# suvajit-patra/sl-hwgat

Measured on AMD Instinct MI355X. Metric: clips/sec fwd+bwd at B=64 T=128 J=67; %HBM roofline; 1->8 GPU scaling, higher is better.
Workload: dtype f32

## Files before the change

### sl-hwgat_amd/csrc/gemm_f32_tn256.hip

```cpp
#include <stdlib.h>
#include <type_traits>
#include "common.h"
#include "fused_ops.h"
#include "gemm_f32.h"
#include "gemm_dispatch.h"

namespace {

constexpr int BT = 256, TM = 16, NST = 3;
constexpr int STG = 2 * TM * BT;

constexpr int SG_MFMA = 0x008, SG_VALU = 0x002, SG_VMEM_RD = 0x020, SG_DS_RD = 0x100, SG_DS_WR = 0x200;

template <int NVM = 0>
__device__ __forceinline__ void pin8() {
#pragma unroll
    for (int q = 0; q < 8; ++q) {
        if (q < 4) __builtin_amdgcn_sched_group_barrier(SG_DS_RD, 1, 0);
        if constexpr (NVM > 0) __builtin_amdgcn_sched_group_barrier(SG_VMEM_RD, NVM, 0);
        __builtin_amdgcn_sched_group_barrier(SG_MFMA, 4, 0);
    }
}
template <int NA, int NB>
__device__ __forceinline__ void pin_commit() {
#pragma unroll
    for (int i = 0; i < 4; ++i) {
        if constexpr (NA > 0) __builtin_amdgcn_sched_group_barrier(SG_VALU, NA, 0);
        __builtin_amdgcn_sched_group_barrier(SG_DS_WR, 1, 0);
        __builtin_amdgcn_sched_group_barrier(SG_DS_RD, 1, 0);
        __builtin_amdgcn_sched_group_barrier(SG_MFMA, 4, 0);
        if constexpr (NB > 0) __builtin_amdgcn_sched_group_barrier(SG_VALU, NB, 0);
        __builtin_amdgcn_sched_group_barrier(SG_DS_WR, 1, 0);
        __builtin_amdgcn_sched_group_barrier(SG_MFMA, 4, 0);
    }
}

#ifdef HWGAT_LAB
__device__ unsigned long long* g_tn256_stamps = nullptr;
#define TN256_STAMP(i) do { if (g_tn256_stamps && threadIdx.x == 0) g_tn256_stamps[blockIdx.x * 2 + (i)] = __builtin_amdgcn_s_memtime(); } while (0)
#else
#define TN256_STAMP(i) do {} while (0)
#endif

template <int PRO, bool BLN, bool SLAB = false>
__global__ __launch_bounds__(256, 1) void gemm_tn256_k(TnArgs p, float* __restrict__ ws = nullptr) {
    HWGAT_RESOLVE_SEED1(p);
    __shared__ __attribute__((aligned(16))) float sm[NST * STG];
    const int tid = threadIdx.x, lane = tid & 63, wave = tid >> 6;
    const int lq = lane & 31, hh = lane >> 5;
    const int wn = wave >> 1, wk = wave & 1;
    const int tiles_k = p.K / BT, n_tiles = (p.N / BT) * tiles_k;
    const int xcd = blockIdx.x & 7, j = blockIdx.x >> 3;
    const int tile = j % n_tiles;
    const int split = (j / n_tiles) * 8 + xcd;
    if (split >= p.n_split) return;
    const int n0 = (tile / tiles_k) * BT, k0 = (tile % tiles_k) * BT;
    const int64_t r_begin = (int64_t)split * p.rows_per_split;
    const int64_t r_end = r_begin + p.rows_per_split < p.M ? r_begin + p.rows_per_split : p.M;
    if (r_begin >= r_end) return;
    const int n_it = (int)((r_end - r_begin) / TM);
    TN256_STAMP(0);

    const int lrow = tid >> 6, lc4 = (tid & 63) * 4;
    const uint32_t pro_th = drop_thresh(p.pro_p);
    const float pro_sc = 1.0f / (1.0f - p.pro_p);
    f32x4 ra[2][4], rb[2][4];
    f32x2 bms[2][4];
    f32x4 colsum = {0.f, 0.f, 0.f, 0.f};
    f32x4 lg = {1.f, 1.f, 1.f, 1.f}, lb = {0.f, 0.f, 0.f, 0.f};
    if constexpr (BLN) {
        lg = *reinterpret_cast<const f32x4*>(p.gamma + k0 + lc4);
        lb = *reinterpret_cast<const f32x4*>(p.beta + k0 + lc4);
    }
    int oa[4], ob[4];
#pragma unroll
    for (int i = 0; i < 4; ++i) { oa[i] = ((lrow + 4 * i) * p.N + lc4) * 4; ob[i] = ((lrow + 4 * i) * p.K + lc4) * 4; }
    auto issue = [&](auto QC, int it) {
        constexpr int Q = decltype(QC)::value;
        const int64_t r0 = r_begin + (int64_t)it * TM;
        const auto da = __builtin_amdgcn_make_buffer_rsrc((void*)(p.A + r0 * p.N + n0), 0, 0x7fffffff, 0x00020000);
        const auto db = __builtin_amdgcn_make_buffer_rsrc((void*)(p.B + r0 * p.K + k0), 0, 0x7fffffff, 0x00020000);
#pragma unroll
        for (int i = 0; i < 4; ++i) {
            ra[Q][i] = __builtin_bit_cast(f32x4, __builtin_amdgcn_raw_buffer_load_b128(da, oa[i], 0, 0));
            rb[Q][i] = __builtin_bit_cast(f32x4, __builtin_amdgcn_raw_buffer_load_b128(db, ob[i], 0, 0));
            if constexpr (BLN) {
                const auto dm = __builtin_amdgcn_make_buffer_rsrc((void*)(p.mean + r0), 0, 0x7fffffff, 0x00020000);
                const auto ds = __builtin_amdgcn_make_buffer_rsrc((void*)(p.rstd + r0), 0, 0x7fffffff, 0x00020000);
                bms[Q][i].x = __builtin_bit_cast(float, __builtin_amdgcn_raw_buffer_load_b32(dm, (lrow + 4 * i) * 4, 0, 0));
                bms[Q][i].y = __builtin_bit_cast(float, __builtin_amdgcn_raw_buffer_load_b32(ds, (lrow + 4 * i) * 4, 0, 0));
            }
        }
    };
    auto commit_a = [&](auto QC, int so, int it, float live, int i) {
        constexpr int Q = decltype(QC)::value;
        f32x4 a = ra[Q][i];
        if constexpr (PRO == PRO_DROP) {
            const int64_t r0 = r_begin + (int64_t)it * TM + lrow;
            a *= drop_keep4(p.pro_seed, (uint64_t)(r0 + 4 * i) * p.N + n0 + lc4, pro_th, pro_sc);
        }
        colsum += a * live;
        *reinterpret_cast<f32x4*>(sm + so * STG + (lrow + 4 * i) * BT + lc4) = a;
    };
    auto commit_b = [&](auto QC, int so, int i) {
        constexpr int Q = decltype(QC)::value;
        f32x4 b = rb[Q][i];
        if constexpr (BLN) {
            f32x2 ms = bms[Q][i];
            asm("" : "+v"(ms));
            b = (b - ms.x) * ms.y * lg + lb;
        }
        *reinterpret_cast<f32x4*>(sm + so * STG + TM * BT + (lrow + 4 * i) * BT + lc4) = b;
    };
    auto commit = [&](auto QC, int so, int it, float live) {
#pragma unroll
        for (int i = 0; i < 4; ++i) { commit_a(QC, so, it, live, i); commit_b(QC, so, i); }
    };

    f32x16 acc[4][4];
#pragma unroll
    for (int i = 0; i < 4; ++i)
#pragma unroll
        for (int jj = 0; jj < 4; ++jj)
#pragma unroll
            for (int e = 0; e < 16; ++e) acc[i][jj][e] = 0.f;

    struct Chunk { f32x4 a[2], b[2]; };
    auto fetch1 = [&](Chunk& c, int so, int ch, int j) {
        const int e = j >> 1;
        const int ro = (2 * (2 * ch + e) + hh) * BT + 4 * lq;
        const float* src = sm + so * STG + ((j & 1) ? TM * BT + wk * 128 : wn * 128) + ro;
        const f32x4 v = *reinterpret_cast<const f32x4*>(__builtin_assume_aligned(src, 16));
        if (j & 1) c.b[e] = v; else c.a[e] = v;
    };
    auto fetch = [&](Chunk& c, int so, int ch) {
#pragma unroll
        for (int j = 0; j < 4; ++j) fetch1(c, so, ch, j);
    };
    auto mfma_chunk = [&](const Chunk& c) {
#pragma unroll
        for (int e = 0; e < 2; ++e)
#pragma unroll
            for (int i = 0; i < 4; ++i)
#pragma unroll
                for (int jj = 0; jj < 4; ++jj)
                    acc[i][jj] = __builtin_amdgcn_mfma_f32_32x32x2f32(c.a[e][i], c.b[e][jj], acc[i][jj], 0, 0, 0);
    };
    Chunk c0, c1;
    constexpr int NV_A = PRO == PRO_DROP ? 52 : 5, NV_B = BLN ? 9 : 1;
    auto stage_body = [&](auto PARC, int it, int st, int st1, int st2) {
        constexpr int PAR = decltype(PARC)::value;
        using Q = std::integral_constant<int, PAR>;
        const int it2 = it + 2 < n_it ? it + 2 : n_it - 1;
        const float live = it + 2 < n_it ? 1.0f : 0.0f;
        issue(std::integral_constant<int, PAR ^ 1>{}, it + 3 < n_it ? it + 3 : n_it - 1);
        fetch(c1, st, 1);
        mfma_chunk(c0);
        pin8<BLN ? 2 : 1>();
        __builtin_amdgcn_sched_barrier(0);
        fetch(c0, st, 2);
        mfma_chunk(c1);
        pin8<>();
        __builtin_amdgcn_sched_barrier(0);
#pragma unroll
        for (int i = 0; i < 4; ++i) {
            commit_a(Q{}, st2, it2, live, i);
            fetch1(c1, st, 3, i);
            commit_b(Q{}, st2, i);
        }
        mfma_chunk(c0);
        pin_commit<NV_A, NV_B>();
        __builtin_amdgcn_sched_barrier(0);
        fetch(c0, st1, 0);
        mfma_chunk(c1);
        pin8<>();
        __builtin_amdgcn_sched_barrier(0);
        __syncthreads();
    };
    using P0 = std::integral_constant<int, 0>;
    using P1 = std::integral_constant<int, 1>;

    issue(P0{}, 0);
    commit(P0{}, 0, 0, 1.0f);
    issue(P1{}, 1);
    commit(P1{}, 1, 1, 1.0f);
    issue(P0{}, 2 < n_it ? 2 : n_it - 1);
    __syncthreads();
    fetch(c0, 0, 0);
#pragma nounroll
    for (int it = 0, s0 = 0, s1 = 1, s2 = 2; it < n_it; it += 2) {
        stage_body(P0{}, it, s0, s1, s2);
        stage_body(P1{}, it + 1, s1, s2, s0);
        const int t = s0; s0 = s2; s2 = s1; s1 = t;
    }

    const bool det = p.det_dw != nullptr;
    float* dwo = det ? p.det_dw + (int64_t)split * p.N * p.K : p.dW;
    if constexpr (SLAB) {
        float* slab = ws + ((int64_t)split * n_tiles + tile) * 65536 + wave * 16384 + lane * 4;
#pragma unroll
        for (int i = 0; i < 4; ++i)
#pragma unroll
            for (int jj = 0; jj < 4; ++jj)
#pragma unroll
                for (int q = 0; q < 4; ++q) {
                    const f32x4 v = {acc[i][jj][4 * q], acc[i][jj][4 * q + 1], acc[i][jj][4 * q + 2], acc[i][jj][4 * q + 3]};
                    *reinterpret_cast<f32x4*>(slab + ((i * 4 + jj) * 4 + q) * 256) = v;
                }
    } else {
#pragma unroll
        for (int i = 0; i < 4; ++i)
#pragma unroll
            for (int jj = 0; jj < 4; ++jj)
#pragma unroll
                for (int r = 0; r < 16; ++r) {
                    const int n = n0 + wn * 128 + 4 * crow(r, hh) + i;
                    const int k = k0 + wk * 128 + 4 * lq + jj;
                    HWGAT_TN_ACC(det, dwo, (int64_t)n * p.K + k, acc[i][jj][r]);
                }
    }
    if (p.db != nullptr && k0 == 0) {
        float* red = sm;
        __syncthreads();
        *reinterpret_cast<f32x4*>(red + lrow * BT + lc4) = colsum;
        __syncthreads();
        if (tid < BT) HWGAT_TN_ACC(det, det ? p.det_db + (int64_t)split * p.N : p.db, n0 + tid, red[tid] + red[BT + tid] + red[2 * BT + tid] + red[3 * BT + tid]);
    }
    TN256_STAMP(1);
}

__global__ __launch_bounds__(256) void tn256_reduce_k(const float* __restrict__ ws, float* __restrict__ dW, int n_split,
                                                      int n_tiles, int tiles_k, int K) {
    const int tile = blockIdx.x >> 8;
    const int idx = (blockIdx.x & 255) * 256 + threadIdx.x;
    const float* src = ws + (int64_t)tile * 65536 + idx;
    const int64_t step = (int64_t)n_tiles * 65536;
    float s = 0.f;
    int sp = 0;
    for (; sp + 8 <= n_split; sp += 8) {
        float v[8];
#pragma unroll
        for (int j = 0; j < 8; ++j) v[j] = src[(sp + j) * step];
#pragma unroll
        for (int j = 0; j < 8; ++j) s += v[j];
    }
    for (; sp < n_split; ++sp) s += src[sp * step];
    const int e = idx & 3, lane = (idx >> 2) & 63, q = (idx >> 8) & 3, t = (idx >> 10) & 15, wave = idx >> 14;
    const int i = t >> 2, jj = t & 3, lq = lane & 31, hh = lane >> 5, wn = wave >> 1, wk = wave & 1;
    const int n0 = (tile / tiles_k) * BT, k0 = (tile % tiles_k) * BT;
    dW[(int64_t)(n0 + wn * 128 + 4 * crow(4 * q + e, hh) + i) * K + k0 + wk * 128 + 4 * lq + jj] += s;
}

}

static void tn256_split(int64_t M, int n_tiles, int& n_split, int64_t& rows_per_split) {
    static const int min_rounds = [] { const char* e = lab_env("HWGAT_TN_ROUNDS"); return e ? atoi(e) : 1; }();
    const TnSplit sp = tn_m_split(M, n_tiles, 256, TM, 2 * TM, min_rounds);
    n_split = sp.n_split;
    rows_per_split = sp.rows_per_split;
}

int64_t hwgat_tn256_ws_floats(int64_t M, int N, int K) {
    if (N % BT || K % BT || M % (2 * TM)) return 0;
    const int n_tiles = (N / BT) * (K / BT);
    int n_split;
    int64_t rows;
    tn256_split(M, n_tiles, n_split, rows);
    return (int64_t)n_split * n_tiles * 65536;
}

int hwgat_launch_tn256(TnArgs a, hipStream_t st, float* ws, int64_t ws_floats) {
    if (a.N % BT || a.K % BT || a.M % (2 * TM)) return HWGAT_ESHAPE;
    const int n_tiles = (a.N / BT) * (a.K / BT);
    tn256_split(a.M, n_tiles, a.n_split, a.rows_per_split);
    if (a.det_dw) {
        if (a.n_split > a.det_cap) return HWGAT_ESHAPE;
        ws = nullptr;
    }
    const int grid = ((a.n_split + 7) / 8) * 8 * n_tiles;
    const bool drop = a.pro_p > 0.f, ln = a.mean != nullptr;
    if (drop && ln) return HWGAT_ESHAPE;
    if (ws && ws_floats >= (int64_t)a.n_split * n_tiles * 65536) {
        if (drop) gemm_tn256_k<PRO_DROP, false, true><<<grid, 256, 0, st>>>(a, ws);
        else if (ln) gemm_tn256_k<PRO_NONE, true, true><<<grid, 256, 0, st>>>(a, ws);
        else gemm_tn256_k<PRO_NONE, false, true><<<grid, 256, 0, st>>>(a, ws);
        tn256_reduce_k<<<n_tiles * 256, 256, 0, st>>>(ws, a.dW, a.n_split, n_tiles, a.K / BT, a.K);
        HWGAT_LAUNCH_CHECK();
    }
    if (drop) gemm_tn256_k<PRO_DROP, false><<<grid, 256, 0, st>>>(a);
    else if (ln) gemm_tn256_k<PRO_NONE, true><<<grid, 256, 0, st>>>(a);
    else gemm_tn256_k<PRO_NONE, false><<<grid, 256, 0, st>>>(a);
    HWGAT_LAUNCH_CHECK();
}

#ifdef HWGAT_LAB
extern "C" int hwgat_lab_tn256_stamps(void* buf) {
    return hipMemcpyToSymbol(HIP_SYMBOL(g_tn256_stamps), &buf, sizeof(buf)) == hipSuccess ? 0 : HWGAT_EINVAL;
}
#endif
```

### sl-hwgat_amd/csrc/gemm_f32_tnw.hip

```cpp
#include <type_traits>
#include "common.h"
#include "fused_ops.h"
#include "gemm_f32.h"

namespace {

constexpr int TM = 16, NST = 3;

constexpr int SG_MFMA = 0x008, SG_VMEM_RD = 0x020, SG_DS_RD = 0x100, SG_DS_WR = 0x200;

template <int MPG, int M1, int N1, int M2, int N2>
__device__ __forceinline__ void il8() {
#pragma unroll
    for (int q = 0; q < 8; ++q) {
        __builtin_amdgcn_sched_group_barrier(SG_MFMA, MPG, 0);
        if constexpr (N1 > 0) __builtin_amdgcn_sched_group_barrier(M1, N1, 0);
        if constexpr (N2 > 0) __builtin_amdgcn_sched_group_barrier(M2, N2, 0);
    }
}

template <int TN, int TK, int WN, int PRO, bool BLN>
__global__ __launch_bounds__(256, 1) void gemm_tnw_k(TnArgs p, float* __restrict__ ws) {
    HWGAT_RESOLVE_SEED1(p);
    constexpr int WK = 4 / WN, IN = TN / WN / 32, JK = TK / WK / 32;
    constexpr int NA = TN / 64, NB = TK / 64;
    constexpr int STG = TM * (TN + TK);
    constexpr int CP = (256 % (TN / 4)) == 0 ? 1 : 3;
    static_assert(TN % 64 == 0 && TK % 64 == 0 && (256 * CP) % (TN / 4) == 0, "tile");
    static_assert(!BLN || 256 % (TK / 4) == 0, "LayerNorm on B: one column group per thread");
    static_assert(IN * JK * 16 <= 192 && IN * WN * 32 == TN && JK * WK * 32 == TK, "sub-tile");
    __shared__ __attribute__((aligned(16))) float sm[NST * STG];
    const int tid = threadIdx.x, lane = tid & 63, wave = tid >> 6;
    const int lq = lane & 31, hh = lane >> 5;
    const int wn = wave / WK, wk = wave % WK;
    const int split = blockIdx.x;
    if (split >= p.n_split) return;
    const int64_t r_begin = (int64_t)split * p.rows_per_split;
    const int64_t r_end = r_begin + p.rows_per_split < p.M ? r_begin + p.rows_per_split : p.M;
    if (r_begin >= r_end) return;
    const int n_it = (int)((r_end - r_begin) / TM);

    const uint32_t pro_th = drop_thresh(p.pro_p);
    const float pro_sc = 1.0f / (1.0f - p.pro_p);
    f32x4 ra[2][NA], rb[2][NB];
    float bm[2][NB], bs[2][NB];
    f32x4 colsum[CP];
#pragma unroll
    for (int j = 0; j < CP; ++j) colsum[j] = f32x4{0.f, 0.f, 0.f, 0.f};
    f32x4 lg = {1.f, 1.f, 1.f, 1.f}, lb = {0.f, 0.f, 0.f, 0.f};
    constexpr int BPR = TK / 4;
    if constexpr (BLN) {
        lg = *reinterpret_cast<const f32x4*>(p.gamma + (tid % BPR) * 4);
        lb = *reinterpret_cast<const f32x4*>(p.beta + (tid % BPR) * 4);
    }
    auto issue = [&](auto QC, int it) {
        constexpr int Q = decltype(QC)::value;
        const int64_t r0 = r_begin + (int64_t)it * TM;
        const float* a = p.A + r0 * TN + tid * 4;
        const float* b = p.B + r0 * TK + tid * 4;
#pragma unroll
        for (int i = 0; i < NA; ++i) ra[Q][i] = *reinterpret_cast<const f32x4*>(a + i * 1024);
#pragma unroll
        for (int i = 0; i < NB; ++i) {
            rb[Q][i] = *reinterpret_cast<const f32x4*>(b + i * 1024);
            if constexpr (BLN) {
                const int64_t row = r0 + (tid + 256 * i) / BPR;
                bm[Q][i] = p.mean[row];
                bs[Q][i] = p.rstd[row];
            }
        }
    };
    auto commit = [&](auto QC, int stage, int it, float live) {
        constexpr int Q = decltype(QC)::value;
        float* As = sm + stage * STG + tid * 4;
        float* Bs = As + TM * TN;
        const uint64_t e0 = (uint64_t)(r_begin + (int64_t)it * TM) * TN + tid * 4;
#pragma unroll
        for (int i = 0; i < NA; ++i) {
            f32x4 a = ra[Q][i];
            if constexpr (PRO == PRO_DROP) a *= drop_keep4(p.pro_seed, e0 + i * 1024, pro_th, pro_sc);
            colsum[i % CP] += a * live;
            *reinterpret_cast<f32x4*>(As + i * 1024) = a;
        }
#pragma unroll
        for (int i = 0; i < NB; ++i) {
            f32x4 b = rb[Q][i];
            if constexpr (BLN) b = (b - bm[Q][i]) * bs[Q][i] * lg + lb;
            *reinterpret_cast<f32x4*>(Bs + i * 1024) = b;
        }
    };

    f32x16 acc[IN][JK];
#pragma unroll
    for (int i = 0; i < IN; ++i)
#pragma unroll
        for (int jj = 0; jj < JK; ++jj)
#pragma unroll
            for (int e = 0; e < 16; ++e) acc[i][jj][e] = 0.f;

    struct Chunk { float a[2][IN], b[2][JK]; };
    auto fetch = [&](Chunk& c, int stage, int ch) {
        const float* As = sm + stage * STG + wn * (IN * 32) + lq;
        const float* Bs = sm + stage * STG + TM * TN + wk * (JK * 32) + lq;
#pragma unroll
        for (int e = 0; e < 2; ++e) {
            const int row = 2 * (2 * ch + e) + hh;
#pragma unroll
            for (int i = 0; i < IN; ++i) c.a[e][i] = As[row * TN + 32 * i];
#pragma unroll
            for (int jj = 0; jj < JK; ++jj) c.b[e][jj] = Bs[row * TK + 32 * jj];
        }
    };
    auto mfma_chunk = [&](const Chunk& c) {
#pragma unroll
        for (int e = 0; e < 2; ++e)
#pragma unroll
            for (int i = 0; i < IN; ++i)
#pragma unroll
                for (int jj = 0; jj < JK; ++jj)
                    acc[i][jj] = __builtin_amdgcn_mfma_f32_32x32x2f32(c.a[e][i], c.b[e][jj], acc[i][jj], 0, 0, 0);
    };
    constexpr int MPG = 2 * IN * JK / 8, RPG = (2 * (IN + JK) + 7) / 8;
    constexpr int LPG = (NA + NB + (BLN ? 2 * NB : 0) + 7) / 8, WPG = (NA + NB + 7) / 8;
    static_assert(MPG * 8 == 2 * IN * JK, "MFMAs per chunk");
    Chunk c0, c1;
    auto stage_body = [&](auto PARC, int it) {
        constexpr int PAR = decltype(PARC)::value;
        const int st = it % NST;
        issue(std::integral_constant<int, PAR ^ 1>{}, it + 3 < n_it ? it + 3 : n_it - 1);
        fetch(c1, st, 1);
        mfma_chunk(c0);
        il8<MPG, SG_DS_RD, RPG, SG_VMEM_RD, LPG>();
        __builtin_amdgcn_sched_barrier(0);
        fetch(c0, st, 2);
        mfma_chunk(c1);
        il8<MPG, SG_DS_RD, RPG, 0, 0>();
        __builtin_amdgcn_sched_barrier(0);
        fetch(c1, st, 3);
        mfma_chunk(c0);
        commit(std::integral_constant<int, PAR>{}, (it + 2) % NST, it + 2 < n_it ? it + 2 : n_it - 1, it + 2 < n_it ? 1.0f : 0.0f);
        il8<MPG, SG_DS_RD, RPG, SG_DS_WR, WPG>();
        __builtin_amdgcn_sched_barrier(0);
        fetch(c0, (it + 1) % NST, 0);
        mfma_chunk(c1);
        il8<MPG, SG_DS_RD, RPG, 0, 0>();
        __builtin_amdgcn_sched_barrier(0);
        __syncthreads();
    };
    using P0 = std::integral_constant<int, 0>;
    using P1 = std::integral_constant<int, 1>;

    issue(P0{}, 0);
    commit(P0{}, 0, 0, 1.0f);
    issue(P1{}, 1);
    commit(P1{}, 1, 1, 1.0f);
    issue(P0{}, 2 < n_it ? 2 : n_it - 1);
    __syncthreads();
    fetch(c0, 0, 0);
    for (int it = 0; it < n_it; it += 2) {
        stage_body(P0{}, it);
        stage_body(P1{}, it + 1);
    }

    const bool det = p.det_dw != nullptr;
    if (ws != nullptr) {
        float* slab = ws + (int64_t)split * (TN * TK) + wave * (IN * JK * 1024) + lane * 4;
#pragma unroll
        for (int i = 0; i < IN; ++i)
#pragma unroll
            for (int jj = 0; jj < JK; ++jj)
#pragma unroll
                for (int q = 0; q < 4; ++q) {
                    const f32x4 v = {acc[i][jj][4 * q], acc[i][jj][4 * q + 1], acc[i][jj][4 * q + 2], acc[i][jj][4 * q + 3]};
                    *reinterpret_cast<f32x4*>(slab + ((i * JK + jj) * 4 + q) * 256) = v;
                }
    } else {
        float* dwo = det ? p.det_dw + (int64_t)split * (TN * TK) : p.dW;
#pragma unroll
        for (int i = 0; i < IN; ++i)
#pragma unroll
            for (int jj = 0; jj < JK; ++jj)
#pragma unroll
                for (int r = 0; r < 16; ++r) {
                    const int n = wn * (IN * 32) + i * 32 + crow(r, hh);
                    const int k = wk * (JK * 32) + jj * 32 + lq;
                    HWGAT_TN_ACC(det, dwo, n * TK + k, acc[i][jj][r]);
                }
    }
    if (p.db != nullptr) {
        constexpr int SL = 1024 * CP / TN;
        float* red = sm;
#pragma unroll
        for (int j = 0; j < CP; ++j) *reinterpret_cast<f32x4*>(red + (tid + 256 * j) * 4) = colsum[j];
        __syncthreads();
        for (int c = tid; c < TN; c += 256) {
            float s = 0.f;
#pragma unroll
            for (int q = 0; q < SL; ++q) s += red[q * TN + c];
            HWGAT_TN_ACC(det, det ? p.det_db + (int64_t)split * TN : p.db, c, s);
        }
    }
}

template <int TN, int TK, int WN>
__global__ __launch_bounds__(256) void tnw_reduce_k(const float* __restrict__ ws, float* __restrict__ dW, int n_split) {
    constexpr int WK = 4 / WN, IN = TN / WN / 32, JK = TK / WK / 32;
    const int idx = blockIdx.x * 256 + threadIdx.x;
    const float* src = ws + idx;
    float s = 0.f;
    int sp = 0;
    for (; sp + 8 <= n_split; sp += 8) {
        float v[8];
#pragma unroll
        for (int j = 0; j < 8; ++j) v[j] = src[(int64_t)(sp + j) * (TN * TK)];
#pragma unroll
        for (int j = 0; j < 8; ++j) s += v[j];
    }
    for (; sp < n_split; ++sp) s += src[(int64_t)sp * (TN * TK)];
    const int e = idx & 3, lane = (idx >> 2) & 63, q = (idx >> 8) & 3, t = (idx >> 10) % (IN * JK), wave = idx / (IN * JK * 1024);
    const int i = t / JK, jj = t % JK, lq = lane & 31, hh = lane >> 5, wn = wave / WK, wk = wave % WK;
    dW[(wn * (IN * 32) + i * 32 + crow(4 * q + e, hh)) * TK + wk * (JK * 32) + jj * 32 + lq] += s;
}

void tnw_split(int64_t M, int& n_split, int64_t& rows_per_split) {
    int64_t want = 256;
    const int64_t max_split = M / (TM * 16) > 0 ? M / (TM * 16) : 1;
    if (want > max_split) want = max_split;
    int64_t rows = (M + want - 1) / want;
    rows = (rows + 2 * TM - 1) / (2 * TM) * (2 * TM);
    n_split = (int)((M + rows - 1) / rows);
    rows_per_split = rows;
}

template <int TN, int TK, int WN>
int launch_shape(const TnArgs& a, hipStream_t st, float* ws) {
    const bool drop = a.pro_p > 0.f, ln = a.mean != nullptr;
    if (drop) gemm_tnw_k<TN, TK, WN, PRO_DROP, false><<<a.n_split, 256, 0, st>>>(a, ws);
    else if (ln) gemm_tnw_k<TN, TK, WN, PRO_NONE, true><<<a.n_split, 256, 0, st>>>(a, ws);
    else gemm_tnw_k<TN, TK, WN, PRO_NONE, false><<<a.n_split, 256, 0, st>>>(a, ws);
    if (ws) tnw_reduce_k<TN, TK, WN><<<TN * TK / 256, 256, 0, st>>>(ws, a.dW, a.n_split);
    HWGAT_LAUNCH_CHECK();
}

}

bool hwgat_tnw_takes(int64_t M, int N, int K, float pro_p, const float* mean) {
    if (M <= 0 || M % (2 * TM) || (pro_p > 0.f && mean)) return false;
    if (N == 128 && K == 128) return pro_p == 0.f;
    return (N == 256 && K == 128) || (N == 128 && K == 256) || (N == 384 && K == 128);
}

int64_t hwgat_tnw_ws_floats(int64_t M, int N, int K) {
    if (!hwgat_tnw_takes(M, N, K, 0.f, nullptr)) return 0;
    int n_split;
    int64_t rows;
    tnw_split(M, n_split, rows);
    return (int64_t)n_split * N * K;
}

int hwgat_launch_tnw(TnArgs a, hipStream_t st, float* ws, int64_t ws_floats) {
    if (!hwgat_tnw_takes(a.M, a.N, a.K, a.pro_p, a.mean)) return HWGAT_ESHAPE;
    tnw_split(a.M, a.n_split, a.rows_per_split);
    if (a.det_dw) {
        if (a.n_split > a.det_cap) return HWGAT_ESHAPE;
        ws = nullptr;
    }
    if (ws && ws_floats < (int64_t)a.n_split * a.N * a.K) ws = nullptr;
    if (a.N == 128 && a.K == 128) return launch_shape<128, 128, 2>(a, st, ws);
    if (a.N == 256 && a.K == 128) return launch_shape<256, 128, 2>(a, st, ws);
    if (a.N == 128 && a.K == 256) return launch_shape<128, 256, 2>(a, st, ws);
    return launch_shape<384, 128, 2>(a, st, ws);
}
```

Measured before the change: 662.1.

## Load LN stats once per quad with DPP broadcast; vectorize tnw LDS fragment reads

In the 256-tile TN kernel, the per-row mean/rstd loads are cut from eight scalar loads per stage to two. Each lane loads one value and the values are shared across the quad with DPP broadcasts, and the schedule pins are adjusted to match. In the tnw kernel, global loads move to buffer loads with immediate offsets. The MFMA operand index mapping is permuted so each lane reads contiguous LDS fragments with vector loads, and the dW writeback and reduce indices are remapped to match. This reduces VMEM and LDS instruction counts but adds DPP ops, and the permuted layout could change LDS bank conflicts.

```diff
diff --git a/sl-hwgat_amd/csrc/gemm_f32_tn256.hip b/sl-hwgat_amd/csrc/gemm_f32_tn256.hip
--- a/sl-hwgat_amd/csrc/gemm_f32_tn256.hip
+++ b/sl-hwgat_amd/csrc/gemm_f32_tn256.hip
@@ -12,12 +12,15 @@
 
 constexpr int SG_MFMA = 0x008, SG_VALU = 0x002, SG_VMEM_RD = 0x020, SG_DS_RD = 0x100, SG_DS_WR = 0x200;
 
-template <int NVM = 0>
+template <int NVM = 0, int NX = 0>
 __device__ __forceinline__ void pin8() {
 #pragma unroll
     for (int q = 0; q < 8; ++q) {
         if (q < 4) __builtin_amdgcn_sched_group_barrier(SG_DS_RD, 1, 0);
-        if constexpr (NVM > 0) __builtin_amdgcn_sched_group_barrier(SG_VMEM_RD, NVM, 0);
+        if constexpr (NVM > 0) {
+            if (q < NX) __builtin_amdgcn_sched_group_barrier(SG_VMEM_RD, NVM + 1, 0);
+            else __builtin_amdgcn_sched_group_barrier(SG_VMEM_RD, NVM, 0);
+        }
         __builtin_amdgcn_sched_group_barrier(SG_MFMA, 4, 0);
     }
 }
@@ -32,6 +35,16 @@
         if constexpr (NB > 0) __builtin_amdgcn_sched_group_barrier(SG_VALU, NB, 0);
         __builtin_amdgcn_sched_group_barrier(SG_DS_WR, 1, 0);
         __builtin_amdgcn_sched_group_barrier(SG_MFMA, 4, 0);
+    }
+}
+
+__device__ __forceinline__ float quad_bcast(float v, int i) {
+    const int x = __builtin_bit_cast(int, v);
+    switch (i) {
+        case 0: return __builtin_bit_cast(float, __builtin_amdgcn_update_dpp(0, x, 0x00, 0xf, 0xf, true));
+        case 1: return __builtin_bit_cast(float, __builtin_amdgcn_update_dpp(0, x, 0x55, 0xf, 0xf, true));
+        case 2: return __builtin_bit_cast(float, __builtin_amdgcn_update_dpp(0, x, 0xaa, 0xf, 0xf, true));
+        default: return __builtin_bit_cast(float, __builtin_amdgcn_update_dpp(0, x, 0xff, 0xf, 0xf, true));
     }
 }
 
@@ -65,7 +78,8 @@
     const uint32_t pro_th = drop_thresh(p.pro_p);
     const float pro_sc = 1.0f / (1.0f - p.pro_p);
     f32x4 ra[2][4], rb[2][4];
-    f32x2 bms[2][4];
+    float bmv[2], bsv[2];
+    const int os = (lrow + 4 * (lane & 3)) * 4;
     f32x4 colsum = {0.f, 0.f, 0.f, 0.f};
     f32x4 lg = {1.f, 1.f, 1.f, 1.f}, lb = {0.f, 0.f, 0.f, 0.f};
     if constexpr (BLN) {
@@ -80,16 +94,16 @@
         const int64_t r0 = r_begin + (int64_t)it * TM;
         const auto da = __builtin_amdgcn_make_buffer_rsrc((void*)(p.A + r0 * p.N + n0), 0, 0x7fffffff, 0x00020000);
         const auto db = __builtin_amdgcn_make_buffer_rsrc((void*)(p.B + r0 * p.K + k0), 0, 0x7fffffff, 0x00020000);
+        if constexpr (BLN) {
+            const auto dm = __builtin_amdgcn_make_buffer_rsrc((void*)(p.mean + r0), 0, 0x7fffffff, 0x00020000);
+            const auto ds = __builtin_amdgcn_make_buffer_rsrc((void*)(p.rstd + r0), 0, 0x7fffffff, 0x00020000);
+            bmv[Q] = __builtin_bit_cast(float, __builtin_amdgcn_raw_buffer_load_b32(dm, os, 0, 0));
+            bsv[Q] = __builtin_bit_cast(float, __builtin_amdgcn_raw_buffer_load_b32(ds, os, 0, 0));
+        }
 #pragma unroll
         for (int i = 0; i < 4; ++i) {
             ra[Q][i] = __builtin_bit_cast(f32x4, __builtin_amdgcn_raw_buffer_load_b128(da, oa[i], 0, 0));
             rb[Q][i] = __builtin_bit_cast(f32x4, __builtin_amdgcn_raw_buffer_load_b128(db, ob[i], 0, 0));
-            if constexpr (BLN) {
-                const auto dm = __builtin_amdgcn_make_buffer_rsrc((void*)(p.mean + r0), 0, 0x7fffffff, 0x00020000);
-                const auto ds = __builtin_amdgcn_make_buffer_rsrc((void*)(p.rstd + r0), 0, 0x7fffffff, 0x00020000);
-                bms[Q][i].x = __builtin_bit_cast(float, __builtin_amdgcn_raw_buffer_load_b32(dm, (lrow + 4 * i) * 4, 0, 0));
-                bms[Q][i].y = __builtin_bit_cast(float, __builtin_amdgcn_raw_buffer_load_b32(ds, (lrow + 4 * i) * 4, 0, 0));
-            }
         }
     };
     auto commit_a = [&](auto QC, int so, int it, float live, int i) {
@@ -106,9 +120,11 @@
         constexpr int Q = decltype(QC)::value;
         f32x4 b = rb[Q][i];
         if constexpr (BLN) {
-            f32x2 ms = bms[Q][i];
-            asm("" : "+v"(ms));
-            b = (b - ms.x) * ms.y * lg + lb;
+            const float mu = quad_bcast(bmv[Q], i), rs = quad_bcast(bsv[Q], i);
+            f32x4 t = b - mu;
+#pragma unroll
+            for (int e = 0; e < 4; ++e) { float te = t[e] * rs; asm("" : "+v"(te)); t[e] = te; }
+            b = t * lg + lb;
         }
         *reinterpret_cast<f32x4*>(sm + so * STG + TM * BT + (lrow + 4 * i) * BT + lc4) = b;
     };
@@ -147,7 +163,7 @@
                     acc[i][jj] = __builtin_amdgcn_mfma_f32_32x32x2f32(c.a[e][i], c.b[e][jj], acc[i][jj], 0, 0, 0);
     };
     Chunk c0, c1;
-    constexpr int NV_A = PRO == PRO_DROP ? 52 : 5, NV_B = BLN ? 9 : 1;
+    constexpr int NV_A = PRO == PRO_DROP ? 52 : 5, NV_B = BLN ? 12 : 1;
     auto stage_body = [&](auto PARC, int it, int st, int st1, int st2) {
         constexpr int PAR = decltype(PARC)::value;
         using Q = std::integral_constant<int, PAR>;
@@ -156,7 +172,7 @@
         issue(std::integral_constant<int, PAR ^ 1>{}, it + 3 < n_it ? it + 3 : n_it - 1);
         fetch(c1, st, 1);
         mfma_chunk(c0);
-        pin8<BLN ? 2 : 1>();
+        pin8<1, BLN ? 2 : 0>();
         __builtin_amdgcn_sched_barrier(0);
         fetch(c0, st, 2);
         mfma_chunk(c1);
diff --git a/sl-hwgat_amd/csrc/gemm_f32_tnw.hip b/sl-hwgat_amd/csrc/gemm_f32_tnw.hip
--- a/sl-hwgat_amd/csrc/gemm_f32_tnw.hip
+++ b/sl-hwgat_amd/csrc/gemm_f32_tnw.hip
@@ -53,20 +53,25 @@
         lg = *reinterpret_cast<const f32x4*>(p.gamma + (tid % BPR) * 4);
         lb = *reinterpret_cast<const f32x4*>(p.beta + (tid % BPR) * 4);
     }
+    const int ot = tid * 16;
+    int os[NB];
+#pragma unroll
+    for (int i = 0; i < NB; ++i) os[i] = ((tid + 256 * i) / BPR) * 4;
     auto issue = [&](auto QC, int it) {
         constexpr int Q = decltype(QC)::value;
         const int64_t r0 = r_begin + (int64_t)it * TM;
-        const float* a = p.A + r0 * TN + tid * 4;
-        const float* b = p.B + r0 * TK + tid * 4;
-#pragma unroll
-        for (int i = 0; i < NA; ++i) ra[Q][i] = *reinterpret_cast<const f32x4*>(a + i * 1024);
+        const auto da = __builtin_amdgcn_make_buffer_rsrc((void*)(p.A + r0 * TN), 0, 0x7fffffff, 0x00020000);
+        const auto db = __builtin_amdgcn_make_buffer_rsrc((void*)(p.B + r0 * TK), 0, 0x7fffffff, 0x00020000);
+#pragma unroll
+        for (int i = 0; i < NA; ++i) ra[Q][i] = __builtin_bit_cast(f32x4, __builtin_amdgcn_raw_buffer_load_b128(da, ot, i * 4096, 0));
 #pragma unroll
         for (int i = 0; i < NB; ++i) {
-            rb[Q][i] = *reinterpret_cast<const f32x4*>(b + i * 1024);
+            rb[Q][i] = __builtin_bit_cast(f32x4, __builtin_amdgcn_raw_buffer_load_b128(db, ot, i * 4096, 0));
             if constexpr (BLN) {
-                const int64_t row = r0 + (tid + 256 * i) / BPR;
-                bm[Q][i] = p.mean[row];
-                bs[Q][i] = p.rstd[row];
+                const auto dm = __builtin_amdgcn_make_buffer_rsrc((void*)(p.mean + r0), 0, 0x7fffffff, 0x00020000);
+                const auto ds = __builtin_amdgcn_make_buffer_rsrc((void*)(p.rstd + r0), 0, 0x7fffffff, 0x00020000);
+                bm[Q][i] = __builtin_bit_cast(float, __builtin_amdgcn_raw_buffer_load_b32(dm, os[i], 0, 0));
+                bs[Q][i] = __builtin_bit_cast(float, __builtin_amdgcn_raw_buffer_load_b32(ds, os[i], 0, 0));
             }
         }
     };
@@ -99,16 +104,32 @@
             for (int e = 0; e < 16; ++e) acc[i][jj][e] = 0.f;
 
     struct Chunk { float a[2][IN], b[2][JK]; };
+    auto frag = [](float* dst, const float* src, auto NC) {
+        constexpr int NF = decltype(NC)::value;
+        if constexpr (NF % 4 == 0) {
+#pragma unroll
+            for (int v = 0; v < NF / 4; ++v) {
+                const f32x4 t = *reinterpret_cast<const f32x4*>(__builtin_assume_aligned(src + 4 * v, 16));
+#pragma unroll
+                for (int u = 0; u < 4; ++u) dst[4 * v + u] = t[u];
+            }
+        } else {
+#pragma unroll
+            for (int v = 0; v < NF / 2; ++v) {
+                const f32x2 t = *reinterpret_cast<const f32x2*>(__builtin_assume_aligned(src + 2 * v, 8));
+                dst[2 * v] = t.x;
+                dst[2 * v + 1] = t.y;
+            }
+        }
+    };
     auto fetch = [&](Chunk& c, int stage, int ch) {
-        const float* As = sm + stage * STG + wn * (IN * 32) + lq;
-        const float* Bs = sm + stage * STG + TM * TN + wk * (JK * 32) + lq;
+        const float* As = sm + stage * STG + wn * (IN * 32) + IN * lq;
+        const float* Bs = sm + stage * STG + TM * TN + wk * (JK * 32) + JK * lq;
 #pragma unroll
         for (int e = 0; e < 2; ++e) {
             const int row = 2 * (2 * ch + e) + hh;
-#pragma unroll
-            for (int i = 0; i < IN; ++i) c.a[e][i] = As[row * TN + 32 * i];
-#pragma unroll
-            for (int jj = 0; jj < JK; ++jj) c.b[e][jj] = Bs[row * TK + 32 * jj];
+            frag(c.a[e], As + row * TN, std::integral_constant<int, IN>{});
+            frag(c.b[e], Bs + row * TK, std::integral_constant<int, JK>{});
         }
     };
     auto mfma_chunk = [&](const Chunk& c) {
@@ -182,8 +203,8 @@
             for (int jj = 0; jj < JK; ++jj)
 #pragma unroll
                 for (int r = 0; r < 16; ++r) {
-                    const int n = wn * (IN * 32) + i * 32 + crow(r, hh);
-                    const int k = wk * (JK * 32) + jj * 32 + lq;
+                    const int n = wn * (IN * 32) + IN * crow(r, hh) + i;
+                    const int k = wk * (JK * 32) + JK * lq + jj;
                     HWGAT_TN_ACC(det, dwo, n * TK + k, acc[i][jj][r]);
                 }
     }
@@ -219,7 +240,7 @@
     for (; sp < n_split; ++sp) s += src[(int64_t)sp * (TN * TK)];
     const int e = idx & 3, lane = (idx >> 2) & 63, q = (idx >> 8) & 3, t = (idx >> 10) % (IN * JK), wave = idx / (IN * JK * 1024);
     const int i = t / JK, jj = t % JK, lq = lane & 31, hh = lane >> 5, wn = wave / WK, wk = wave % WK;
-    dW[(wn * (IN * 32) + i * 32 + crow(4 * q + e, hh)) * TK + wk * (JK * 32) + jj * 32 + lq] += s;
+    dW[(wn * (IN * 32) + IN * crow(4 * q + e, hh) + i) * TK + wk * (JK * 32) + JK * lq + jj] += s;
 }
 
 void tnw_split(int64_t M, int& n_split, int64_t& rows_per_split) {
```

Result: no change. 663.2 (median of 2 runs) (+0.2%).
